# py-lidbox/lidbox

Measured on AMD Instinct MI355X. Metric: utterances/sec (16kHz x 2s) log-mel + x-vector train step, higher is better.
Workload: dtype f32; 1 GPU; log-mel + x-vector 4-lang train step, bs=256 per GPU, fp32 (BASELINE configs[1]); reference_model=lidbox.models.xvector, global_batch=256, per_gpu_batch=256, samples_per_utt=32000, frames=198, mel=40, languages=4, optimizer=Adam(1e-3, eps=1e-7), parallelism=dp1, grad_buckets=1, grad_sync=none, hip_graph=True, resident_batches=4, feature_prefetch=False

## Files before the change

### lidbox_amd/csrc/gemm.hip

```cpp
#include <stdlib.h>

#include <atomic>

#include "gemm_shared.h"
#include "gemm_sk.h"
#include <string.h>
#include "gemm_dma.h"
#include "gemm_dma8.h"
#include "gemm_tuned.h"

namespace {

constexpr int BK = 16;
#define LBX_ROWS_BOUNDS(BM, BN) __launch_bounds__(256, ((BM) * (BN) >= 16384 ? 3 : ((BM) * (BN) >= 8192 ? 6 : 8)))
#define LBX_TN_BOUNDS(BM, BN) __launch_bounds__(256, ((BM) * (BN) >= 16384 ? 3 : 1))

template <int ROWS, bool ALIGNED, int NT = 256>
struct KInnerLoader {
    static constexpr int F4R = BK / 4;
    static constexpr int RPP = NT / F4R;
    static constexpr int PASSES = ROWS >= RPP ? ROWS / RPP : 1;
    static constexpr bool PARTIAL = ROWS < RPP;
    static constexpr int LD = ROWS + 8 / F4R;
    float4 v[PASSES];
// ... 621 lines not shown

inline int dma_mode() {
    if (const char* e = getenv("LIDBOX_GEMM_DMA")) return atoi(e);
    return 1;
}

template <int BM, int BN, bool B_KINNER>
void launch_rows_dma_t(dim3 grid, hipStream_t st, RowsD Ad, const float* Bm, long ldb, RowsOutD Co, float* P, long m_beg, long m_end,
                       int K, int N, int epi, const float* aux, int tiles_n, unsigned ntiles, int kps, const DmaStream& sp, const ReduceJobs& rj) {
    hipLaunchKernelGGL((gemm_rows_dma_kernel<BM, BN, B_KINNER>), grid, dim3(256), 0, st, Ad, Bm, ldb, Co, P, m_beg, m_end, K, N, epi,
                       aux, tiles_n, ntiles, kps, sp, rj);
}

inline long carry_cap() {
    if (const char* e = getenv("LIDBOX_GEMM_CARRY_BLOCKS")) { const long v = atol(e); if (v >= 8) return v; }
    return 96;
}
struct Carry {
    const ReduceJob* jobs = nullptr;
    int njobs = 0;
    bool carried = false;
};

constexpr int DMA_STREAM_MIN_STEPS = 8;
constexpr int DMA_STREAM_MAX_G = 8;
struct DmaStreamPlan {
    int g = 0;
    long whole = 0, rem = 0;
    size_t ws_need = 0;
};
inline DmaStreamPlan dma_stream_plan(int bm, int bn, long M, int N, int K) {
    DmaStreamPlan pl;
    int force = -1;
    if (const char* e = getenv("LIDBOX_GEMM_STREAM_TAIL")) force = atoi(e);
    if (force == 0) return pl;
    const long tiles = lbx_cdiv(M, bm) * lbx_cdiv(N, bn);
    const long rem = tiles % NUM_CU;
    if (tiles < NUM_CU || rem == 0) return pl;
    const int nk = (int)lbx_cdiv(K, SK_BK);
    int best = 1;
    double best_cost = 1.0;
    for (int g = 2; g <= DMA_STREAM_MAX_G && nk / g >= DMA_STREAM_MIN_STEPS; ++g) {
        const double cost = (double)lbx_cdiv(rem * g, (long)NUM_CU) / g + 0.03 + 0.01 * g;
        if (cost < best_cost - 1e-9) { best_cost = cost; best = g; }
    }
    if (force > 1 && nk / force >= 2 && force <= 64) best = force;
    else if (best_cost > 0.9) return pl;
    if (best < 2) return pl;
    pl.g = best; pl.rem = rem; pl.whole = tiles - rem;
    pl.ws_need = SK_COUNTER_BYTES + (size_t)rem * best * bm * bn * sizeof(float);
    return pl;
}

template <bool B_KINNER>
int launch_rows_range(const RowsChoice& ch, bool al, RowsD Ad, const float* Bm, long ldb, RowsOutD Co, long m_beg,
                      long m_end, int K, int N, int epi, const float* aux, float* P, hipStream_t st, bool dma_ok = false,
                      const DmaStreamPlan* stream = nullptr, void* ws = nullptr, Carry* carry = nullptr) {
    const long Msub = m_end - m_beg;
    if (Msub <= 0) return LIDBOX_OK;
    const int tiles_n = (int)lbx_cdiv(N, ch.bn);
    const long ntiles = lbx_cdiv(Msub, ch.bm) * tiles_n;
    dim3 grid((unsigned)ntiles, (unsigned)ch.splits);
    if (g_last_launches[0] == 0) { g_first_tile[0] = ch.bm; g_first_tile[1] = ch.bn; }
    ++g_last_launches[(ch.bm == g_first_tile[0] && ch.bn == g_first_tile[1]) ? 0 : 1];
    if (ch.splits > 1) ++g_last_launches[2];
#define LBX_ROWS(BM_, BN_) launch_rows_t<BM_, BN_, B_KINNER>(al, grid, st, Ad, Bm, ldb, Co, P, m_beg, m_end, K, N, epi, aux, tiles_n, (unsigned)ntiles, ch.k_per_split)
#define LBX_ROWS8(BM_, BN_) launch_rows8_t<BM_, BN_, B_KINNER>(al, grid, st, Ad, Bm, ldb, Co, P, m_beg, m_end, K, N, epi, aux, tiles_n, (unsigned)ntiles, ch.k_per_split)
#define LBX_ROWS_DMA(BM_, BN_) launch_rows_dma_t<BM_, BN_, B_KINNER>(grid, st, Ad, Bm, ldb, Co, P, m_beg, m_end, K, N, epi, aux, tiles_n, ntiles_k, ch.k_per_split, sp, rj)
    if (dma_ok && al && dma_mode() != 0) {
        g_last_family = 1;
        DmaStream sp;
        const bool dma8 = ch.waves == 8 && ch.bm == 128;
        ReduceJobs rj;
        if (carry && !carry->carried && carry->njobs > 0) {
            rj = pack_carry(carry->jobs, carry->njobs, carry_cap());
            carry->carried = rj.total > 0;
        }
        unsigned ntiles_k = (unsigned)ntiles;
        if (stream && stream->g > 1 && ch.splits == 1) {
            sp.pieces = (unsigned)(stream->rem * stream->g);
            sp.npad = (sp.pieces + 7u) & ~7u;
            sp.g = stream->g;
            sp.first_tile = (unsigned)stream->whole;
            sp.epoch = sk_next_epoch();
            sp.counters = (unsigned*)ws;
            sp.slabs = (float*)((char*)ws + SK_COUNTER_BYTES);
            ntiles_k = (unsigned)stream->whole;
            grid.x = sp.npad + ntiles_k;
        }
        grid.x += rj.total;
        if (dma8) {
            g_last_family = 3;
            if (ch.bn == 128)
                hipLaunchKernelGGL((gemm_rows_dma8_kernel<128, B_KINNER>), grid, dim3(512), 0, st, Ad, Bm, ldb, Co, P, m_beg, m_end, K, N, epi, aux, tiles_n,
                                   ntiles_k, ch.k_per_split, sp, rj);
            else
                hipLaunchKernelGGL((gemm_rows_dma8_kernel<64, B_KINNER>), grid, dim3(512), 0, st, Ad, Bm, ldb, Co, P, m_beg, m_end, K, N, epi, aux, tiles_n,
                                   ntiles_k, ch.k_per_split, sp, rj);
        } else
        if (ch.bm == 128 && ch.bn == 128) LBX_ROWS_DMA(128, 128);
        else if (ch.bm == 128) LBX_ROWS_DMA(128, 64);
        else if (ch.bn == 128) LBX_ROWS_DMA(64, 128);
        else LBX_ROWS_DMA(64, 64);
    } else
    if (ch.waves == 8 && ch.bm == 128 && ch.bn == 128) LBX_ROWS8(128, 128);
    else if (ch.waves == 8 && ch.bm == 128 && ch.bn == 64) LBX_ROWS8(128, 64);
    else if (ch.bm == 128 && ch.bn == 128) LBX_ROWS(128, 128);
    else if (ch.bm == 128) LBX_ROWS(128, 64);
    else if (ch.bn == 128) LBX_ROWS(64, 128);
    else LBX_ROWS(64, 64);
#undef LBX_ROWS
#undef LBX_ROWS8
    LBX_LAUNCH_OK();
    if (ch.splits > 1) {
        long g = lbx_cdiv(Msub * N, 256);
        if (g > 2048) g = 2048;
        hipLaunchKernelGGL(rows_reduce_kernel, dim3((unsigned)g), dim3(256), 0, st, (const float*)P, ch.splits, m_beg,
                           Msub, N, Co, epi, aux);
        LBX_LAUNCH_OK();
    }
    return LIDBOX_OK;
}

inline int cand_index(int bm, int bn) { return bm == 128 ? (bn == 128 ? 0 : 1) : (bn == 128 ? 2 : 3); }

template <bool B_KINNER>
int launch_rows(lidbox_rows_t A, const float* Bm, long ldb, lidbox_rows_out_t Cd, int K, int N, int epi,
                const float* aux, void* ws, size_t ws_bytes, hipStream_t st, Carry* carry = nullptr) {
    const long M = (long)A.batch * A.rows_per_batch;
    g_last_launches[0] = g_last_launches[1] = g_last_launches[2] = 0;
    g_last_family = 0;
    if (M == 0 || N == 0) return LIDBOX_OK;
    const size_t wsb = ws ? ws_bytes : 0;
    const RowsChoice ch = choose_rows_env(B_KINNER ? 1 : 0, M, N, K, wsb);
    const bool al = rows_aligned(A) && K % 4 == 0 && aligned16(Bm) && ldb % 4 == 0 &&
                    (B_KINNER ? true : N % 4 == 0);
    RowsD Ad = to_dev(A);
    RowsOutD Co{Cd.base, Cd.batch_stride, Cd.row_stride, Cd.batch, Cd.rows_per_batch};
    float* P = (float*)ws;

    if (al && !getenv("LIDBOX_GEMM_PLAN") && aligned16(ws) && !sk_tuned_out(B_KINNER ? 1 : 0, M, N, K) &&
        sk_b_extent_ok(B_KINNER, K, N, ldb)) {
        const bool has_mask_ = epi == LIDBOX_EPI_RELU_MASK || epi == LIDBOX_EPI_ACCUM_RELU_MASK;
        const bool skp_ok = skp_mode() != 0 && (Cd.batch == 1 || Cd.rows_per_batch >= 32) && N % 4 == 0 && aligned16(Cd.base) &&
                            Cd.row_stride % 4 == 0 && (Cd.batch == 1 || Cd.batch_stride % 4 == 0) && (!has_mask_ || aligned16(aux)) &&
                            skp_policy(B_KINNER ? 1 : 0, M, N, K);
        if (skp_ok) {
            const SkRows sk = sk_rows_plan(B_KINNER ? 1 : 0, M, N, K, true);
            if (sk.ok && wsb >= sk.ws_need && sk_extent_ok(A, K)) {
                sk_set_lds_attr();
                g_last_launches[0] = 1;
                g_last_family = 2;
                g_first_tile[0] = SK_BM; g_first_tile[1] = SK_BN;
                unsigned* counters = (unsigned*)ws;
                float* slabs = (float*)((char*)ws + SK_COUNTER_BYTES);
                float* dummy = slabs + (size_t)sk.P * 2 * SK_SLAB;
                const bool has_mask = epi == LIDBOX_EPI_RELU_MASK || epi == LIDBOX_EPI_ACCUM_RELU_MASK;
                const bool accum = epi == LIDBOX_EPI_ACCUM || epi == LIDBOX_EPI_ACCUM_RELU_MASK || epi == LIDBOX_EPI_ACCUM_RELU;
                const unsigned ep = sk_next_epoch();
#define LBX_SKP(MASK_, ACC_)                                                                                                \
    hipLaunchKernelGGL((gemm_skp_rows_kernel<B_KINNER, MASK_, ACC_>), dim3(sk.P), dim3(256), (MASK_ || ACC_) ? SKP_LDS_BYTES : SK_LDS_BYTES, st, Ad, Bm, ldb, Co, M, K, \
                       N, epi, aux, sk.pl, ep, counters, slabs, dummy)
                if (has_mask && accum) LBX_SKP(true, true);
                else if (has_mask) LBX_SKP(true, false);
                else if (accum) LBX_SKP(false, true);
                else LBX_SKP(false, false);
#undef LBX_SKP
                LBX_LAUNCH_OK();
                return LIDBOX_OK;
            }
        }
        const SkRows sk = sk_rows_plan(B_KINNER ? 1 : 0, M, N, K);
        if (sk.ok && wsb >= sk.ws_need && sk_extent_ok(A, K)) {
            sk_set_lds_attr();
            g_last_launches[0] = 1;
            g_last_family = 2;
            g_first_tile[0] = SK_BM; g_first_tile[1] = SK_BN;
            unsigned* counters = (unsigned*)ws;
            float* slabs = (float*)((char*)ws + SK_COUNTER_BYTES);
            hipLaunchKernelGGL((gemm_sk_rows_kernel<B_KINNER>), dim3(sk.P), dim3(256), SK_LDS_BYTES, st, Ad, Bm, ldb, Co, M, K, N, epi,
                               aux, sk.pl, sk_next_epoch(), counters, slabs);
            LBX_LAUNCH_OK();
            return LIDBOX_OK;
        }
    }

    const bool dma_ok = al && sk_extent_ok(A, K) && sk_b_extent_ok(B_KINNER, K, N, ldb);
    if (dma_ok && dma_mode() != 0 && ch.splits == 1 && aligned16(ws)) {
        const DmaStreamPlan spl = dma_stream_plan(ch.bm, ch.bn, M, N, K);
        if (spl.g > 1 && wsb >= spl.ws_need)
            return launch_rows_range<B_KINNER>(ch, al, Ad, Bm, ldb, Co, 0, M, K, N, epi, aux, P, st, dma_ok, &spl, ws, carry);
    }
    const bool no_tail_split = ch.no_tail_split || getenv("LIDBOX_GEMM_NO_TAIL_SPLIT") != nullptr;
    if (!no_tail_split && ch.splits == 1) {
        const int tiles_n = (int)lbx_cdiv(N, ch.bn);
        const long tiles_m = lbx_cdiv(M, ch.bm);
        const long wgs = tiles_m * tiles_n;
        const long rounds = wgs / NUM_CU;
        if (rounds >= 1 && wgs % NUM_CU != 0) {
            const long main_tiles_m = rounds * NUM_CU / tiles_n;
            const long m_main = main_tiles_m * ch.bm;
            const long m_rem = M - m_main;
            if (main_tiles_m >= 1 && m_rem > 0) {
                const RowsChoice rem = choose_rows(B_KINNER ? 1 : 0, m_rem, N, K, wsb);
                const int c = cand_index(ch.bm, ch.bn), cr = cand_index(rem.bm, rem.bn);
                const double ksteps = (double)lbx_cdiv(K, BK);
                const double whole = launch_cost(c, wgs, ksteps);
                double split = launch_cost(c, main_tiles_m * tiles_n, ksteps) + 4.0 +
                               launch_cost(cr, lbx_cdiv(m_rem, rem.bm) * lbx_cdiv(N, rem.bn) * rem.splits,
                                           (double)rem.k_per_split / BK);
                if (rem.splits > 1) split += 5.0 + (double)m_rem * N * 4.0 * (rem.splits + 1) / 3.0e6;
                if (split < 0.97 * whole) {
                    int rc = launch_rows_range<B_KINNER>(ch, al, Ad, Bm, ldb, Co, 0, m_main, K, N, epi, aux, P, st, dma_ok, nullptr, nullptr, carry);
                    if (rc) return rc;
                    return launch_rows_range<B_KINNER>(rem, al, Ad, Bm, ldb, Co, m_main, M, K, N, epi, aux, P, st, dma_ok);
                }
            }
        }
    }
    return launch_rows_range<B_KINNER>(ch, al, Ad, Bm, ldb, Co, 0, M, K, N, epi, aux, P, st, dma_ok, nullptr, nullptr, carry);
}

struct TnPlan {
    int bm, bn, splits;
    long rows_per_split;
};

TnPlan tn_plan(long M, int K1, int N) {
    if (const char* f = getenv("LIDBOX_GEMM_TN_PLAN")) {
        int bm = 0, bn = 0;
        long sp = 0;
        if (sscanf(f, "%d,%d,%ld", &bm, &bn, &sp) == 3 && (bm == 64 || bm == 128) && (bn == 64 || bn == 128) && sp >= 1) {
            const long rps = lbx_cdiv(lbx_cdiv(M, sp), BK) * BK;
            return TnPlan{bm, bn, (int)lbx_cdiv(M, rps), rps};
        }
    }
    if (const TunedGemm* t = tuned_gemm(2, M, N, K1)) {
        const long rps = lbx_cdiv(lbx_cdiv(M, (long)t->splits), BK) * BK;
        return TnPlan{t->bm, t->bn, (int)lbx_cdiv(M, rps), rps};
    }
    TnPlan best{128, 128, 1, M};
    double best_cost = 1e30;
    for (int c = 0; c < 4; ++c) {
        const int bm = CAND[c][0], bn = CAND[c][1];
        const long tiles = lbx_cdiv(K1, bm) * lbx_cdiv(N, bn);
        for (long target = NUM_CU; target <= 8 * NUM_CU; target += NUM_CU / 2) {
            long s = target / tiles;
            if (s < 1) s = 1;
            const long max_s = lbx_cdiv(M, 4 * BK);
            if (s > max_s) s = max_s;
            if (s < 1) s = 1;
            long rps = lbx_cdiv(lbx_cdiv(M, s), BK) * BK;
            s = lbx_cdiv(M, rps);
            double cost = launch_cost(c, tiles * s, (double)rps / BK);
            cost += 5.0 + (double)K1 * N * 4.0 * (s + 1) / 3.0e6;
            if (cost < best_cost) { best_cost = cost; best = TnPlan{bm, bn, (int)s, rps}; }
        }
    }
    return best;
}

template <int BM, int BN>
void launch_tn_t(bool al, unsigned grid, hipStream_t st, RowsD A, RowsD Bd, float* P, float* Pc, long M, int K1, int N,
                 int tiles_n, int ntiles, long rps) {
    if (al)
        hipLaunchKernelGGL((gemm_tn_kernel<BM, BN, true>), dim3(grid), dim3(256), 0, st, A, Bd, P, Pc, M, K1, N, tiles_n,
                           ntiles, rps);
    else
        hipLaunchKernelGGL((gemm_tn_kernel<BM, BN, false>), dim3(grid), dim3(256), 0, st, A, Bd, P, Pc, M, K1, N, tiles_n,
                           ntiles, rps);
}

}
// ... 1 lines not shown
extern "C" int lidbox_gemm_plan_query(int kind, long M, int N, int K, size_t workspace_bytes, int* out4) {
    LBX_ARG(out4 && M > 0 && N > 0 && K > 0 && kind >= 0 && kind <= 2, "kind in {0 nn, 1 nt, 2 tn}, positive sizes");
    if (kind == 2) {
        const TnPlan pl = tn_plan(M, K, N);
        out4[0] = pl.bm; out4[1] = pl.bn; out4[2] = pl.splits; out4[3] = (int)pl.rows_per_split;
    } else {
        const RowsChoice ch = choose_rows_env(kind, M, N, K, workspace_bytes);
        out4[0] = ch.bm; out4[1] = ch.bn; out4[2] = ch.splits; out4[3] = ch.k_per_split;
    }
    return LIDBOX_OK;
}

extern "C" int lidbox_gemm_plan_is_stream_k(int kind, long M, int N, int K, size_t workspace_bytes) {
    if (M <= 0 || N <= 0 || K <= 0 || kind < 0 || kind > 2) return 0;
    if (kind == 2) {
        const SkTn t = sk_tn_plan(M, K, N);
        return t.ok && workspace_bytes >= t.ws_need && !sk_tuned_out(2, M, N, K);
    }
    {
        const SkRows r = sk_rows_plan(kind, M, N, K);
        return r.ok && workspace_bytes >= r.ws_need && (kind == 1 || N % 4 == 0) && !sk_tuned_out(kind, M, N, K);
    }
    return LIDBOX_OK;
}

extern "C" int lidbox_gemm_plan_waves(int kind, long M, int N, int K, size_t workspace_bytes) {
    if (M <= 0 || N <= 0 || K <= 0 || kind < 0 || kind > 1) return 4;
    return choose_rows_env(kind, M, N, K, workspace_bytes).waves;
}

extern "C" int lidbox_gemm_last_family(void) { return g_last_family; }

extern "C" int lidbox_gemm_plan_stream_tail(int kind, long M, int N, int K, size_t workspace_bytes) {
    if (M <= 0 || N <= 0 || K <= 0 || kind < 0 || kind > 1 || dma_mode() == 0) return 0;
    if (!getenv("LIDBOX_GEMM_PLAN") && lidbox_gemm_plan_is_stream_k(kind, M, N, K, workspace_bytes)) return 0;
    const RowsChoice ch = choose_rows_env(kind, M, N, K, workspace_bytes);
    if (ch.splits != 1) return 0;
    const DmaStreamPlan spl = dma_stream_plan(ch.bm, ch.bn, M, N, K);
    return (spl.g > 1 && workspace_bytes >= spl.ws_need) ? spl.g : 0;
}

extern "C" int lidbox_gemm_last_launches(int* out3) {
    LBX_ARG(out3, "out3 != NULL");
    out3[0] = g_last_launches[0]; out3[1] = g_last_launches[1]; out3[2] = g_last_launches[2];
    return LIDBOX_OK;
}

extern "C" size_t lidbox_gemm_rows_workspace(long M, int N, int K) {
    if (M <= 0 || N <= 0 || K <= 0) return 0;
    size_t need = 0;
    for (int kind = 0; kind < 2; ++kind) {
        const RowsChoice ch = choose_rows(kind, M, N, K, (size_t)64 << 20);
        if (ch.splits > 1 && (size_t)ch.splits * M * N * sizeof(float) > need) need = (size_t)ch.splits * M * N * sizeof(float);
    }
    for (int bm = 64; bm <= 128; bm += 64)
        for (int bn = 64; bn <= 128; bn += 64) {
            const DmaStreamPlan spl = dma_stream_plan(bm, bn, M, N, K);
            if (spl.g > 1 && spl.ws_need > need) need = spl.ws_need;
        }
    for (int kind = 0; kind < 2; ++kind) {
        const SkRows sk = sk_rows_plan(kind, M, N, K);
        if (sk.ok && sk.ws_need > need) need = sk.ws_need;
        if (skp_mode() != 0 && skp_policy(kind, M, N, K)) {
            const SkRows skp = sk_rows_plan(kind, M, N, K, true);
            if (skp.ok && skp.ws_need > need) need = skp.ws_need;
        }
    }
    return need;
}

extern "C" int lidbox_gemm_nn(lidbox_rows_t A, const float* Bm, long ldb, lidbox_rows_out_t C, int K, int N,
                              int epilogue, const float* aux, void* workspace, size_t workspace_bytes,
                              lidbox_stream_t stream) {
    if (validate_rows_call(__func__, A, Bm, ldb, C, K, N, epilogue, aux, N)) return LIDBOX_E_INVALID;
    return launch_rows<false>(A, Bm, ldb, C, K, N, epilogue, aux, workspace, workspace_bytes, (hipStream_t)stream);
}


extern "C" int lidbox_gemm_nt(lidbox_rows_t A, const float* Bm, long ldb, lidbox_rows_out_t C, int K, int N,
                              int epilogue, const float* aux, void* workspace, size_t workspace_bytes,
                              lidbox_stream_t stream) {
    if (validate_rows_call(__func__, A, Bm, ldb, C, K, N, epilogue, aux, K)) return LIDBOX_E_INVALID;
    return launch_rows<true>(A, Bm, ldb, C, K, N, epilogue, aux, workspace, workspace_bytes, (hipStream_t)stream);
}

extern "C" size_t lidbox_gemm_tn_workspace(int M, int K1, int N) {
    if (M <= 0 || K1 <= 0 || N <= 0) return 0;
    const TnPlan pl = tn_plan(M, K1, N);
    size_t need = ((size_t)pl.splits * K1 * N + (size_t)pl.splits * N) * sizeof(float);
    const SkTn sk = sk_tn_plan(M, K1, N);
    if (sk.ok && sk.ws_need > need) need = sk.ws_need;
    return need;
}

namespace {

int tn_partial_launch(const char* fn, lidbox_rows_t A, lidbox_rows_t Bd, float* Cm, long ldc, int K1, int N, int accumulate,
                      float* bias_grad, void* workspace, size_t workspace_bytes, hipStream_t st, ReduceJob* job) {
    *job = ReduceJob{};
    if (check_rows(fn, A.base, A.batch_stride, A.row_stride, A.batch, A.rows_per_batch)) return LIDBOX_E_INVALID;
    if (check_rows(fn, Bd.base, Bd.batch_stride, Bd.row_stride, Bd.batch, Bd.rows_per_batch)) return LIDBOX_E_INVALID;
    LBX_ARG(Cm && K1 >= 1 && N >= 1 && ldc >= N, "C != NULL, K1, N >= 1, ldc >= N");
    const long M = (long)A.batch * A.rows_per_batch;
    LBX_ARG(M == (long)Bd.batch * Bd.rows_per_batch, "A and B row counts differ");
    LBX_ARG(M >= 1, "M >= 1");
    auto finish = [&](const float* P, const float* Pc, int splits) {
// ... 168 lines not shown
    if (ch_out) *ch_out = ch;
    if (pl_out) *pl_out = pl;
    return true;
}

extern "C" int lidbox_gemm_nt_tn_carry(lidbox_rows_t dY, const float* W, long ldb, lidbox_rows_out_t dX, int Co, int N, int epilogue,
                                       const float* aux, void* ws_nt, size_t ws_nt_bytes, lidbox_rows_t X, float* dW, long ldc, int K1,
                                       int accumulate, float* bias_grad, void* ws_tn, size_t ws_tn_bytes,
                                       const lidbox_reduce_job_t* jobs, int njobs, lidbox_reduce_job_t* job_out, lidbox_stream_t stream) {
    hipStream_t st = (hipStream_t)stream;
    if (job_out) memset(job_out, 0, sizeof *job_out);
    ReduceJob pend[MAX_CARRY];
    const int npend = jobs_in(jobs, njobs, pend);
    LBX_ARG(npend >= 0 && npend < MAX_CARRY, "at most 1 non-empty pending job per call");
    for (int i = 0; i < npend; ++i)
        LBX_ARG((const void*)pend[i].P != ws_nt && (const void*)pend[i].P != ws_tn, "a pending job's slices live in this call's workspaces");
    for (int i = 0; i < npend; ++i) LBX_ARG(pend[i].splits >= 0, "an optimizer-prepare job runs through lidbox_reduce_jobs_run only");
    const long M = (long)dY.batch * dY.rows_per_batch;
    bool pair = dma_mode() != 0 && getenv("LIDBOX_GEMM_NO_PAIR") == nullptr && M >= 1 && N >= 1 && K1 >= 1 && Co >= 1 && W && dW && ws_tn &&
                ws_nt != ws_tn;
    if (pair) {
        if (validate_rows_call(__func__, dY, W, ldb, dX, Co, N, epilogue, aux, Co)) return LIDBOX_E_INVALID;
        if (check_rows(__func__, X.base, X.batch_stride, X.row_stride, X.batch, X.rows_per_batch)) return LIDBOX_E_INVALID;
        LBX_ARG((long)X.batch * X.rows_per_batch == M && ldc >= Co, "X and dY row counts differ, or ldc < Co");
    }
    RowsChoice ch{};
    TnPlan pl{};
    if (pair) {
        const size_t wsb = ws_nt ? ws_nt_bytes : 0;
        const bool al_rows = rows_aligned(dY) && aligned16(W) && ldb % 4 == 0 && sk_extent_ok(dY, Co) && sk_b_extent_ok(true, Co, N, ldb) &&
                             aligned16(ws_nt);
        const bool al_tn = rows_aligned(X) && sk_extent_ok(X, K1) && aligned16(ws_tn);
        pair = al_rows && al_tn && pair_plan(M, Co, N, K1, wsb, ws_tn_bytes, &ch, &pl);
    }
    if (!pair) {
        lidbox_reduce_job_t all[MAX_CARRY];
        for (int i = 0; i < npend; ++i) memcpy(&all[i], &pend[i], sizeof(ReduceJob));
        int rc = lidbox_gemm_tn_partial(X, dY, dW, ldc, K1, Co, accumulate, bias_grad, ws_tn, ws_tn_bytes, &all[npend], stream);
        if (rc) return rc;
        if (ws_nt == ws_tn) {
            rc = lidbox_reduce_jobs_run(all, npend + 1, stream);
            if (rc) return rc;
            return lidbox_gemm_nt(dY, W, ldb, dX, Co, N, epilogue, aux, ws_nt, ws_nt_bytes, stream);
        }
        return lidbox_gemm_nt_carry(dY, W, ldb, dX, Co, N, epilogue, aux, ws_nt, ws_nt_bytes, all, npend + 1, stream);
    }
    PairRows r;
    r.A = to_dev(dY); r.Bm = W; r.ldb = ldb;
    r.Cd = RowsOutD{dX.base, dX.batch_stride, dX.row_stride, dX.batch, dX.rows_per_batch};
    r.P = (float*)ws_nt; r.M = M; r.K = Co; r.N = N; r.epi = epilogue; r.aux = aux;
    r.tiles_n = (int)lbx_cdiv((long)N, 64L);
    r.ntiles = (unsigned)(lbx_cdiv(M, 64L) * r.tiles_n);
    r.k_per_split = ch.k_per_split; r.nx = r.ntiles; r.partial = ch.splits > 1 ? 1 : 0;
    if (ch.splits == 1 && ws_nt) {
        const DmaStreamPlan spl = dma_stream_plan(64, 64, M, N, Co);
        if (spl.g > 1 && ws_nt_bytes >= spl.ws_need) {
            r.sp.pieces = (unsigned)(spl.rem * spl.g);
            r.sp.npad = (r.sp.pieces + 7u) & ~7u;
            r.sp.g = spl.g;
            r.sp.first_tile = (unsigned)spl.whole;
            r.sp.epoch = sk_next_epoch();
            r.sp.counters = (unsigned*)ws_nt;
            r.sp.slabs = (float*)((char*)ws_nt + SK_COUNTER_BYTES);
            r.ntiles = (unsigned)spl.whole;
            r.nx = r.sp.npad + r.ntiles;
        }
    }
    PairTn t;
    t.A = to_dev(X); t.Bd = to_dev(dY);
    t.P = (float*)ws_tn; t.Pc = bias_grad ? t.P + (size_t)pl.splits * K1 * Co : nullptr;
    t.M = M; t.K1 = K1; t.N = Co; t.tiles_n = (int)lbx_cdiv((long)Co, 64L);
    t.ntiles = (int)(lbx_cdiv((long)K1, 64L) * t.tiles_n);
    t.rows_per_split = pl.rows_per_split;
    const unsigned rows_blocks = r.nx * (unsigned)ch.splits;
    ReduceJobs rj;
    if (npend > 0 && getenv("LIDBOX_GEMM_NO_CARRY") == nullptr) rj = pack_carry(pend, npend, carry_cap());
    const unsigned grid = rj.total + rows_blocks + (unsigned)(t.ntiles * pl.splits);
    g_last_launches[0] = 1; g_last_launches[1] = 0; g_last_launches[2] = (job_out ? 0 : 1) + (ch.splits > 1 ? 1 : 0);
    g_last_family = 1;
    g_last_carried = rj.total > 0 ? npend : 0;
    hipLaunchKernelGGL(gemm_nt_tn_pair_kernel, dim3(grid), dim3(256), 0, st, r, t, rows_blocks, rj);
    LBX_LAUNCH_OK();
    if (npend > 0 && rj.total == 0) {
        int rc = run_reduce_jobs(pend, npend, st);
        if (rc) return rc;
    }
    if (ch.splits > 1) {
        long g = lbx_cdiv(M * N, 256);
        if (g > 2048) g = 2048;
        hipLaunchKernelGGL(rows_reduce_kernel, dim3((unsigned)g), dim3(256), 0, st, (const float*)r.P, ch.splits, 0L, M, N, r.Cd, epilogue,
                           aux);
        LBX_LAUNCH_OK();
    }
    if (job_out && reduce_job_vec_ok(t.P, t.Pc, pl.splits, (long)K1 * Co, Co, dW, ldc, bias_grad)) {
        const ReduceJob j = make_reduce_job(t.P, t.Pc, pl.splits, (long)K1 * Co, Co, dW, ldc, accumulate, bias_grad);
        memcpy(job_out, &j, sizeof j);
        return LIDBOX_OK;
    }
    launch_splitk_reduce((const float*)t.P, (const float*)t.Pc, pl.splits, (long)K1 * Co, Co, dW, ldc, accumulate, bias_grad, st);
    LBX_LAUNCH_OK();
    return LIDBOX_OK;
}

extern "C" int lidbox_gemm_nt_tn(lidbox_rows_t dY, const float* W, long ldb, lidbox_rows_out_t dX, int Co, int N, int epilogue,
                                 const float* aux, void* ws_nt, size_t ws_nt_bytes, lidbox_rows_t X, float* dW, long ldc, int K1,
                                 int accumulate, float* bias_grad, void* ws_tn, size_t ws_tn_bytes, lidbox_stream_t stream) {
    return lidbox_gemm_nt_tn_carry(dY, W, ldb, dX, Co, N, epilogue, aux, ws_nt, ws_nt_bytes, X, dW, ldc, K1, accumulate, bias_grad, ws_tn,
                                   ws_tn_bytes, nullptr, 0, nullptr, stream);
}

extern "C" int lidbox_gemm_plan_is_pair(long M, int Co, int N, int K1, size_t ws_nt_bytes, size_t ws_tn_bytes) {
    return pair_plan(M, Co, N, K1, ws_nt_bytes, ws_tn_bytes, nullptr, nullptr) ? 1 : 0;
}

extern "C" size_t lidbox_colsum_workspace(long M, int N) {
    long slices = lbx_cdiv(M, 256);
    if (slices > 128) slices = 128;
    if (slices < 1) slices = 1;
    return (size_t)slices * N * sizeof(float);
}

extern "C" int lidbox_colsum(lidbox_rows_t A, int N, float* out, int accumulate, void* workspace,
                             size_t workspace_bytes, lidbox_stream_t stream) {
    if (check_rows(__func__, A.base, A.batch_stride, A.row_stride, A.batch, A.rows_per_batch)) return LIDBOX_E_INVALID;
    LBX_ARG(out && N >= 1, "out != NULL, N >= 1");
    const long M = (long)A.batch * A.rows_per_batch;
    long slices = lbx_cdiv(M, 256);
    if (slices > 128) slices = 128;
    if (slices < 1) slices = 1;
    LBX_ARG(workspace && workspace_bytes >= (size_t)slices * N * sizeof(float), "workspace too small (lidbox_colsum_workspace)");
    const long rps = lbx_cdiv(M, slices);
    hipStream_t st = (hipStream_t)stream;
    hipLaunchKernelGGL(colsum_stage1, dim3((unsigned)lbx_cdiv(N, 64), (unsigned)slices), dim3(256), 0, st,
                       to_dev(A), M, N, rps, (float*)workspace);
    LBX_LAUNCH_OK();
    hipLaunchKernelGGL(colsum_stage2, dim3((unsigned)lbx_cdiv(N, 256)), dim3(256), 0, st, (const float*)workspace,
                       (int)slices, N, out, accumulate);
    LBX_LAUNCH_OK();
    return LIDBOX_OK;
}
// ... 1 lines not shown
```

### lidbox_amd/csrc/gemm_dma.h

```cpp
#pragma once

#include "gemm_sk.h"

namespace {

constexpr int DMA_STAGES = 3;

template <int ROWS>
struct DmaInner {
    static constexpr int PW = ROWS / 64;
    const float* sb;
    unsigned vo[PW];
    int rd;
    __device__ __forceinline__ void init(const float* base, const long (&roff)[PW], int k0, int lane, int wsub) {
        sb = sk_uniform(base + k0);
        const int chunk = (lane & 3) ^ ((lane >> 4) & 3);
#pragma unroll
        for (int i = 0; i < PW; ++i) vo[i] = (unsigned)((roff[i] + chunk * 4) * 4);
        rd = (wsub * (ROWS / 2) + (lane & 31)) * 16;
    }
    __device__ __forceinline__ void issue(int i, unsigned dst) const { sk_dma_s(sb, vo[i], dst); }
    __device__ __forceinline__ void issue_tail(int i, unsigned dst, int kvalid, int lane) const {
        const int chunk = (lane & 3) ^ ((lane >> 4) & 3);
        const float* p = reinterpret_cast<const float*>(reinterpret_cast<const char*>(sb) + vo[i]);
// ... 13 lines not shown

template <int COLS>
struct DmaOuter {
    static constexpr int PW = COLS / 64;
    static constexpr int LPR = COLS / 4;
    static constexpr int RPP = 64 / LPR;
    const float* sb;
    unsigned vo[PW];
    long step;
    int rd;
    __device__ __forceinline__ void init(const float* base, long ld, int col0, int ncols, int k0, int lane, int wv, int wsub) {
        sb = sk_uniform(base + (long)k0 * ld + col0);
        int c = (lane % LPR) * 4;
        if (col0 + c >= ncols) c = 0;
#pragma unroll
        for (int i = 0; i < PW; ++i) vo[i] = (unsigned)(((long)(RPP * (wv * PW + i) + lane / LPR) * ld + c) * 4);
        step = (long)SK_BK * ld;
        rd = (4 * (lane >> 5)) * COLS + wsub * (COLS / 2) + (lane & 31);
    }
    __device__ __forceinline__ void issue(int i, unsigned dst) const { sk_dma_s(sb, vo[i], dst); }
    __device__ __forceinline__ void issue_tail(int i, unsigned dst, int kvalid, int lane, int wv) const {
        const float* p = reinterpret_cast<const float*>(reinterpret_cast<const char*>(sb) + vo[i]);
        sk_dma_f(RPP * (wv * PW + i) + lane / LPR < kvalid ? p : g_sk_zero, dst);
    }
    __device__ __forceinline__ void advance() { sb += step; }
    template <int NB>
    __device__ __forceinline__ void read(const float* st, int lane, int s2, float (&v)[NB][4]) const {
#pragma unroll
        for (int b = 0; b < NB; ++b)
#pragma unroll
            for (int j = 0; j < 4; ++j) v[b][j] = st[rd + (8 * s2 + j) * COLS + b * 32];
    }
};

template <int MI, int NJ, int J0, int J1>
__device__ __forceinline__ void dma_mma(const float (&a)[MI][4], const float (&b)[NJ][4], f32x16 (&acc)[MI][NJ]) {
#pragma unroll
    for (int j = J0; j < J1; ++j)
#pragma unroll
        for (int bi = 0; bi < MI; ++bi)
#pragma unroll
            for (int bj = 0; bj < NJ; ++bj)
                acc[bi][bj] = __builtin_amdgcn_mfma_f32_32x32x2f32(a[bi][j], b[bj][j], acc[bi][bj], 0, 0, 0);
}

struct DmaStream {
    unsigned npad = 0;
    unsigned pieces = 0;
    int g = 1;
    unsigned first_tile = 0;
    unsigned epoch = 0;
    unsigned* counters = nullptr;
    float* slabs = nullptr;
};

template <int MI, int NJ>
__device__ __forceinline__ void dma_slab_store(float* slab, const f32x16 (&acc)[MI][NJ], int wv, int lane) {
    const __amdgpu_buffer_rsrc_t r = __builtin_amdgcn_make_buffer_rsrc(const_cast<float*>(sk_uniform(slab)), 0, MI * NJ * 4096 * 4, 0x00020000);
#pragma unroll
    for (int bi = 0; bi < MI; ++bi)
#pragma unroll
        for (int bj = 0; bj < NJ; ++bj)
#pragma unroll
            for (int r4 = 0; r4 < 4; ++r4) {
                const f32x4_t x = {acc[bi][bj][4 * r4], acc[bi][bj][4 * r4 + 1], acc[bi][bj][4 * r4 + 2], acc[bi][bj][4 * r4 + 3]};
                __builtin_amdgcn_raw_buffer_store_b128(__builtin_bit_cast(u32x4_t, x), r,
                                                       ((((wv * (MI * NJ) + bi * NJ + bj) * 4 + r4) * 64 + lane) * 4) * 4, 0,  16);
            }
}
template <int MI, int NJ>
__device__ __forceinline__ void dma_slab_add(const float* slab, f32x16 (&acc)[MI][NJ], int wv, int lane) {
    const __amdgpu_buffer_rsrc_t r = __builtin_amdgcn_make_buffer_rsrc(const_cast<float*>(sk_uniform(slab)), 0, MI * NJ * 4096 * 4, 0x00020000);
#pragma unroll
    for (int bi = 0; bi < MI; ++bi)
#pragma unroll
        for (int bj = 0; bj < NJ; ++bj) {
#pragma unroll
            for (int r4 = 0; r4 < 4; ++r4) {
                const f32x4_t x = __builtin_bit_cast(
                    f32x4_t, __builtin_amdgcn_raw_buffer_load_b128(r, ((((wv * (MI * NJ) + bi * NJ + bj) * 4 + r4) * 64 + lane) * 4) * 4, 0,  16));
#pragma unroll
                for (int j = 0; j < 4; ++j) acc[bi][bj][4 * r4 + j] += x[j];
            }
            __builtin_amdgcn_sched_barrier(0);
        }
}

template <int BM, int BN, bool B_KINNER>
__device__ __forceinline__ void rows_dma_body(const RowsD& A, const float* __restrict__ Bm, long ldb, const RowsOutD& Cd, float* __restrict__ P,
                                              long m_beg, long M, int K, int N, int epi, const float* __restrict__ aux, int tiles_n,
                                              unsigned ntiles, int k_per_split, const DmaStream& sp, unsigned bx, unsigned by, int partial,
                                              float* smem) {
    constexpr int MI = BM / 64, NJ = BN / 64;
    constexpr int A_ST = BM * SK_BK, B_ST = SK_BK * BN, ST = A_ST + B_ST;
    constexpr int PA = BM / 64, PB = BN / 64;

    const int tid = threadIdx.x, lane = tid & 63;
    const int wv = __builtin_amdgcn_readfirstlane(tid >> 6);
    const int wm = wv >> 1, wn = wv & 1;
    const unsigned lds0 = __builtin_amdgcn_readfirstlane((unsigned)(size_t)(__attribute__((address_space(3))) void*)smem);
    const int split = (int)by;
    unsigned chunk;
    int kbeg, kend, part = -1;
    unsigned rem_t = 0;
    if (bx < sp.npad) {
        if (bx >= sp.pieces) return;
        rem_t = bx / (unsigned)sp.g;
        part = (int)(bx - rem_t * (unsigned)sp.g);
        chunk = sp.first_tile + rem_t;
        const int nk = (K + SK_BK - 1) / SK_BK;
        kbeg = (part * nk / sp.g) * SK_BK;
        kend = min(K, ((part + 1) * nk / sp.g) * SK_BK);
    } else {
        chunk = xcd_chunk_id(bx - sp.npad, ntiles);
        kbeg = split * k_per_split;
        kend = min(K, kbeg + k_per_split);
    }
    const int tn = chunk % tiles_n;
    const long m0 = m_beg + (long)(chunk / tiles_n) * BM;
    const int n0 = tn * BN;
    const int n = (kend - kbeg + SK_BK - 1) / SK_BK;
    const int ktail = kend - kbeg - (n - 1) * SK_BK;

    DmaInner<BM> oa;
    {
        long roff[PA];
#pragma unroll
        for (int i = 0; i < PA; ++i) {
            long r = m0 + 16 * (wv * PA + i) + (lane >> 2);
            if (r >= M) r = m0;
            roff[i] = row_offset(A, (unsigned)r);
        }
        oa.init(A.base, roff, kbeg, lane, wm);
    }
    DmaInner<BN> obi;
    DmaOuter<BN> obo;
    if (B_KINNER) {
        long roff[PB];
#pragma unroll
        for (int i = 0; i < PB; ++i) {
            long r = n0 + 16 * (wv * PB + i) + (lane >> 2);
            if (r >= N) r = n0;
            roff[i] = r * ldb;
        }
        obi.init(Bm, roff, kbeg, lane, wn);
    } else {
        obo.init(Bm, ldb, n0, N, kbeg, lane, wv, wn);
    }
    f32x16 acc[MI][NJ];
#pragma unroll
    for (int i = 0; i < MI; ++i)
#pragma unroll
        for (int j = 0; j < NJ; ++j)
#pragma unroll
            for (int r = 0; r < 16; ++r) acc[i][j][r] = 0.f;

    auto issue = [&](int pc, int step, int stage) {
        const bool tail = step == n - 1 && ktail < SK_BK;
        if (pc < PA) {
            const unsigned d = lds0 + (unsigned)((stage * ST + (wv * PA + pc) * 256) * 4);
            if (tail) oa.issue_tail(pc, d, ktail, lane);
            else oa.issue(pc, d);
        } else {
            const int q = pc - PA;
            const unsigned d = lds0 + (unsigned)((stage * ST + A_ST + (wv * PB + q) * 256) * 4);
            if (B_KINNER) { if (tail) obi.issue_tail(q, d, ktail, lane); else obi.issue(q, d); }
            else { if (tail) obo.issue_tail(q, d, ktail, lane, wv); else obo.issue(q, d); }
        }
    };
// ... 17 lines not shown
        }
    if (n >= DMA_STAGES - 1) sk_wait_vm<(DMA_STAGES - 2) * NP>();
    else sk_wait_vm<0>();
    __builtin_amdgcn_s_barrier();
    float a0[MI][4], b0[NJ][4], a1[MI][4], b1[NJ][4];
    if (n > 0) {
        ra(smem, 0, a0);
        rb(smem + A_ST, 0, b0);
    }
    int cur = 0;
    for (int t = 0; t < n; ++t) {
        if (t + 1 < n) {
            if (DMA_STAGES >= 4 && t + DMA_STAGES - 2 < n) sk_wait_vm<(DMA_STAGES >= 4 ? (DMA_STAGES - 3) * NP : 0)>();
            else sk_wait_vm<0>();
        }
        __builtin_amdgcn_s_barrier();
        int nxt = cur + 1;
        if (nxt == DMA_STAGES) nxt = 0;
        const bool more = t + DMA_STAGES - 1 < n;
        int tgt = cur + DMA_STAGES - 1;
        if (tgt >= DMA_STAGES) tgt -= DMA_STAGES;
        const float* st = smem + cur * ST;
        dma_mma<MI, NJ, 0, 1>(a0, b0, acc);
        __builtin_amdgcn_sched_barrier(0);
        ra(st, 1, a1);
        rb(st + A_ST, 1, b1);
        __builtin_amdgcn_sched_barrier(0);
        dma_mma<MI, NJ, 1, 2>(a0, b0, acc);
        if (more) issue(0, t + DMA_STAGES - 1, tgt);
        __builtin_amdgcn_sched_barrier(0);
        dma_mma<MI, NJ, 2, 3>(a0, b0, acc);
        if (more) issue(1, t + DMA_STAGES - 1, tgt);
        __builtin_amdgcn_sched_barrier(0);
        dma_mma<MI, NJ, 3, 4>(a0, b0, acc);
        if (more && NP > 2) issue(2, t + DMA_STAGES - 1, tgt);
        __builtin_amdgcn_sched_barrier(0);
        dma_mma<MI, NJ, 0, 1>(a1, b1, acc);
        if (more) {
            if (NP > 3) issue(3, t + DMA_STAGES - 1, tgt);
            next();
        }
        __builtin_amdgcn_sched_barrier(0);
        if (t + 1 < n) {
            const float* sn = smem + nxt * ST;
            ra(sn, 0, a0);
            rb(sn + A_ST, 0, b0);
        }
        __builtin_amdgcn_sched_barrier(0);
        dma_mma<MI, NJ, 1, 4>(a1, b1, acc);
        cur = nxt;
    }
    if (part >= 0) {
        constexpr int SLAB = BM * BN;
        dma_slab_store<MI, NJ>(sp.slabs + (size_t)bx * SLAB, acc, wv, lane);
        asm volatile("s_waitcnt vmcnt(0)" ::: "memory");
        __syncthreads();
        unsigned* flag = reinterpret_cast<unsigned*>(smem);
        if (tid == 0) {
            unsigned old = __hip_atomic_load(sp.counters + rem_t, __ATOMIC_RELAXED, __HIP_MEMORY_SCOPE_AGENT);
            unsigned cnt;
            for (;;) {
                cnt = (old >> 8) == sp.epoch ? (old & 255u) : 0u;
                if (__hip_atomic_compare_exchange_strong(sp.counters + rem_t, &old, (sp.epoch << 8) | (cnt + 1u), __ATOMIC_RELAXED,
                                                         __ATOMIC_RELAXED, __HIP_MEMORY_SCOPE_AGENT))
                    break;
            }
            *flag = cnt;
        }
        __syncthreads();
        if (*flag != (unsigned)(sp.g - 1)) return;
#pragma unroll
        for (int i = 0; i < MI; ++i)
#pragma unroll
            for (int j = 0; j < NJ; ++j)
#pragma unroll
                for (int r = 0; r < 16; ++r) acc[i][j][r] = 0.f;
        for (int q = 0; q < sp.g; ++q)
            dma_slab_add<MI, NJ>(sp.slabs + ((size_t)rem_t * sp.g + q) * SLAB, acc, wv, lane);
        if (tid == 0) __hip_atomic_store(sp.counters + rem_t, 0u, __ATOMIC_RELAXED, __HIP_MEMORY_SCOPE_AGENT);
    }
    store_rows_tile<MI, NJ>(acc, m0, n0, wm, wn, lane, m_beg, M, N, epi, aux, Cd, P, split, 0ull, false, nullptr, nullptr, partial);
}

template <int BM, int BN>
constexpr int dma_stage_floats() { return (BM + BN) * SK_BK; }

template <int BM, int BN, bool B_KINNER>
__global__ __launch_bounds__(256, (BM * BN >= 16384 ? 3 : (BM * BN >= 8192 ? 4 : 6))) void gemm_rows_dma_kernel(
    RowsD A, const float* __restrict__ Bm, long ldb, RowsOutD Cd, float* __restrict__ P, long m_beg, long M, int K, int N, int epi,
    const float* __restrict__ aux, int tiles_n, unsigned ntiles, int k_per_split, DmaStream sp, ReduceJobs rj) {
    __shared__ __attribute__((aligned(16))) float smem[DMA_STAGES * dma_stage_floats<BM, BN>()];
    if (blockIdx.x < rj.total) {
        if (blockIdx.y == 0) reduce_jobs_run(rj, blockIdx.x);
        return;
    }
    rows_dma_body<BM, BN, B_KINNER>(A, Bm, ldb, Cd, P, m_beg, M, K, N, epi, aux, tiles_n, ntiles, k_per_split, sp, blockIdx.x - rj.total,
                                    blockIdx.y, gridDim.y > 1 ? 1 : 0, smem);
}

template <int COLS>
struct DmaOuterRows {
    static constexpr int PW = COLS / 64;
    static constexpr int LPR = COLS / 4;
    static constexpr int RPP = 64 / LPR;
    const float* sb;
    int off[PW];
    unsigned tt[PW];
    int a_step, a_wrap;
    unsigned rpb;
    int mleft[PW];
    int rd;

    __device__ __forceinline__ void init(const RowsD& X, int col0, int ncols, long mbeg, long mend, int lane, int wv, int wsub) {
        sb = sk_uniform(X.base + col0);
        int c = (lane % LPR) * 4;
        if (col0 + c >= ncols) c = 0;
        a_step = (int)(SK_BK * X.rs);
        a_wrap = X.batch == 1 ? 0 : (int)(X.bs - (long)X.rpb * X.rs);
        rpb = X.batch == 1 ? 0xffffffffu : (unsigned)X.rpb;
#pragma unroll
        for (int i = 0; i < PW; ++i) {
            const long m = mbeg + RPP * (wv * PW + i) + lane / LPR;
            const unsigned bq = X.batch == 1 ? 0u : (unsigned)m / rpb;
            tt[i] = (unsigned)m - (X.batch == 1 ? 0u : bq * rpb);
            off[i] = (int)((long)bq * X.bs + (long)tt[i] * X.rs) + c;
            mleft[i] = (int)(mend - m);
        }
        rd = (4 * (lane >> 5)) * COLS + wsub * (COLS / 2) + (lane & 31);
    }
    __device__ __forceinline__ void issue(int i, unsigned dst, bool tail) {
        if (!tail) {
            sk_dma_s(sb, (unsigned)off[i] * 4u, dst);
        } else {
            const float* p = reinterpret_cast<const float*>(reinterpret_cast<const char*>(sb) + (size_t)((unsigned)off[i] * 4u));
            sk_dma_f(mleft[i] > 0 ? p : g_sk_zero, dst);
        }
        mleft[i] -= SK_BK;
        tt[i] += SK_BK;
        off[i] += a_step;
        while (tt[i] >= rpb) { tt[i] -= rpb; off[i] += a_wrap; }
    }
    template <int NB>
    __device__ __forceinline__ void read(const float* st, int lane, int s2, float (&v)[NB][4]) const {
#pragma unroll
        for (int b = 0; b < NB; ++b)
#pragma unroll
            for (int j = 0; j < 4; ++j) v[b][j] = st[rd + (8 * s2 + j) * COLS + b * 32];
    }
};

// ... 151 lines not shown
```

Baseline: 120,200 utterances/s.

## Finish split-K reduction in-kernel via atomic counters instead of separate reduce launch

For 64x64 split-K DMA GEMM launches, each split writes its partial tile into a per-tile slab, and the last split to arrive (found through an epoch-tagged atomic counter) sums all slabs and runs the epilogue. This removes the separate rows_reduce_kernel launch and its full partial-buffer pass. It adds a batched slab-sum helper and requires a larger workspace sizing path. The cost is atomics, serialized summation in the last-arriving block, and extra slab traffic.

Result: slower. 117,400 utterances/s (-2.4%).

```diff
diff --git a/lidbox_amd/csrc/gemm.hip b/lidbox_amd/csrc/gemm.hip
--- a/lidbox_amd/csrc/gemm.hip
+++ b/lidbox_amd/csrc/gemm.hip
@@ -697,10 +697,22 @@
     return pl;
 }
 
+inline size_t split_finish_ws(long tiles, int splits) { return SK_COUNTER_BYTES + (size_t)tiles * splits * 64 * 64 * sizeof(float); }
+inline bool split_finish_ok(const RowsChoice& ch, long tiles, const void* ws, size_t ws_bytes) {
+    return ch.splits > 1 && ch.splits <= 250 && ch.bm == 64 && ch.bn == 64 && ch.waves != 8 && ws && aligned16(ws) &&
+           (size_t)tiles * sizeof(unsigned) <= SK_COUNTER_BYTES && ws_bytes >= split_finish_ws(tiles, ch.splits);
+}
+inline void split_finish_arm(DmaStream& sp, int splits, void* ws) {
+    sp.g = splits;
+    sp.epoch = sk_next_epoch();
+    sp.counters = (unsigned*)ws;
+    sp.slabs = (float*)((char*)ws + SK_COUNTER_BYTES);
+}
+
 template <bool B_KINNER>
 int launch_rows_range(const RowsChoice& ch, bool al, RowsD Ad, const float* Bm, long ldb, RowsOutD Co, long m_beg,
                       long m_end, int K, int N, int epi, const float* aux, float* P, hipStream_t st, bool dma_ok = false,
-                      const DmaStreamPlan* stream = nullptr, void* ws = nullptr, Carry* carry = nullptr) {
+                      const DmaStreamPlan* stream = nullptr, void* ws = nullptr, Carry* carry = nullptr, size_t ws_bytes = 0) {
     const long Msub = m_end - m_beg;
     if (Msub <= 0) return LIDBOX_OK;
     const int tiles_n = (int)lbx_cdiv(N, ch.bn);
@@ -708,7 +720,7 @@
     dim3 grid((unsigned)ntiles, (unsigned)ch.splits);
     if (g_last_launches[0] == 0) { g_first_tile[0] = ch.bm; g_first_tile[1] = ch.bn; }
     ++g_last_launches[(ch.bm == g_first_tile[0] && ch.bn == g_first_tile[1]) ? 0 : 1];
-    if (ch.splits > 1) ++g_last_launches[2];
+    bool reduce = ch.splits > 1;
 #define LBX_ROWS(BM_, BN_) launch_rows_t<BM_, BN_, B_KINNER>(al, grid, st, Ad, Bm, ldb, Co, P, m_beg, m_end, K, N, epi, aux, tiles_n, (unsigned)ntiles, ch.k_per_split)
 #define LBX_ROWS8(BM_, BN_) launch_rows8_t<BM_, BN_, B_KINNER>(al, grid, st, Ad, Bm, ldb, Co, P, m_beg, m_end, K, N, epi, aux, tiles_n, (unsigned)ntiles, ch.k_per_split)
 #define LBX_ROWS_DMA(BM_, BN_) launch_rows_dma_t<BM_, BN_, B_KINNER>(grid, st, Ad, Bm, ldb, Co, P, m_beg, m_end, K, N, epi, aux, tiles_n, ntiles_k, ch.k_per_split, sp, rj)
@@ -732,6 +744,9 @@
             sp.slabs = (float*)((char*)ws + SK_COUNTER_BYTES);
             ntiles_k = (unsigned)stream->whole;
             grid.x = sp.npad + ntiles_k;
+        } else if (split_finish_ok(ch, ntiles, P, ws_bytes)) {
+            split_finish_arm(sp, ch.splits, P);
+            reduce = false;
         }
         grid.x += rj.total;
         if (dma8) {
@@ -757,7 +772,8 @@
 #undef LBX_ROWS
 #undef LBX_ROWS8
     LBX_LAUNCH_OK();
-    if (ch.splits > 1) {
+    if (reduce) {
+        ++g_last_launches[2];
         long g = lbx_cdiv(Msub * N, 256);
         if (g > 2048) g = 2048;
         hipLaunchKernelGGL(rows_reduce_kernel, dim3((unsigned)g), dim3(256), 0, st, (const float*)P, ch.splits, m_beg,
@@ -858,12 +874,12 @@
                 if (split < 0.97 * whole) {
                     int rc = launch_rows_range<B_KINNER>(ch, al, Ad, Bm, ldb, Co, 0, m_main, K, N, epi, aux, P, st, dma_ok, nullptr, nullptr, carry);
                     if (rc) return rc;
-                    return launch_rows_range<B_KINNER>(rem, al, Ad, Bm, ldb, Co, m_main, M, K, N, epi, aux, P, st, dma_ok);
+                    return launch_rows_range<B_KINNER>(rem, al, Ad, Bm, ldb, Co, m_main, M, K, N, epi, aux, P, st, dma_ok, nullptr, nullptr, nullptr, wsb);
                 }
             }
         }
     }
-    return launch_rows_range<B_KINNER>(ch, al, Ad, Bm, ldb, Co, 0, M, K, N, epi, aux, P, st, dma_ok, nullptr, nullptr, carry);
+    return launch_rows_range<B_KINNER>(ch, al, Ad, Bm, ldb, Co, 0, M, K, N, epi, aux, P, st, dma_ok, nullptr, nullptr, carry, wsb);
 }
 
 struct TnPlan {
@@ -971,6 +987,10 @@
     for (int kind = 0; kind < 2; ++kind) {
         const RowsChoice ch = choose_rows(kind, M, N, K, (size_t)64 << 20);
         if (ch.splits > 1 && (size_t)ch.splits * M * N * sizeof(float) > need) need = (size_t)ch.splits * M * N * sizeof(float);
+        if (ch.splits > 1 && ch.bm == 64 && ch.bn == 64) {
+            const size_t fin = split_finish_ws(lbx_cdiv(M, 64L) * lbx_cdiv((long)N, 64L), ch.splits);
+            if (fin > need) need = fin;
+        }
     }
     for (int bm = 64; bm <= 128; bm += 64)
         for (int bn = 64; bn <= 128; bn += 64) {
@@ -1245,6 +1265,11 @@
     r.tiles_n = (int)lbx_cdiv((long)N, 64L);
     r.ntiles = (unsigned)(lbx_cdiv(M, 64L) * r.tiles_n);
     r.k_per_split = ch.k_per_split; r.nx = r.ntiles; r.partial = ch.splits > 1 ? 1 : 0;
+    const bool finish = split_finish_ok(ch, (long)r.ntiles, ws_nt, ws_nt ? ws_nt_bytes : 0);
+    if (finish) {
+        split_finish_arm(r.sp, ch.splits, ws_nt);
+        r.partial = 0;
+    }
     if (ch.splits == 1 && ws_nt) {
         const DmaStreamPlan spl = dma_stream_plan(64, 64, M, N, Co);
         if (spl.g > 1 && ws_nt_bytes >= spl.ws_need) {
@@ -1269,7 +1294,7 @@
     ReduceJobs rj;
     if (npend > 0 && getenv("LIDBOX_GEMM_NO_CARRY") == nullptr) rj = pack_carry(pend, npend, carry_cap());
     const unsigned grid = rj.total + rows_blocks + (unsigned)(t.ntiles * pl.splits);
-    g_last_launches[0] = 1; g_last_launches[1] = 0; g_last_launches[2] = (job_out ? 0 : 1) + (ch.splits > 1 ? 1 : 0);
+    g_last_launches[0] = 1; g_last_launches[1] = 0; g_last_launches[2] = (job_out ? 0 : 1) + (ch.splits > 1 && !finish ? 1 : 0);
     g_last_family = 1;
     g_last_carried = rj.total > 0 ? npend : 0;
     hipLaunchKernelGGL(gemm_nt_tn_pair_kernel, dim3(grid), dim3(256), 0, st, r, t, rows_blocks, rj);
@@ -1278,7 +1303,7 @@
         int rc = run_reduce_jobs(pend, npend, st);
         if (rc) return rc;
     }
-    if (ch.splits > 1) {
+    if (ch.splits > 1 && !finish) {
         long g = lbx_cdiv(M * N, 256);
         if (g > 2048) g = 2048;
         hipLaunchKernelGGL(rows_reduce_kernel, dim3((unsigned)g), dim3(256), 0, st, (const float*)r.P, ch.splits, 0L, M, N, r.Cd, epilogue,
diff --git a/lidbox_amd/csrc/gemm_dma.h b/lidbox_amd/csrc/gemm_dma.h
--- a/lidbox_amd/csrc/gemm_dma.h
+++ b/lidbox_amd/csrc/gemm_dma.h
@@ -89,6 +89,7 @@
     unsigned epoch = 0;
     unsigned* counters = nullptr;
     float* slabs = nullptr;
+    __host__ __device__ bool finishes_splits() const { return npad == 0 && g > 1; }
 };
 
 template <int MI, int NJ>
@@ -104,6 +105,42 @@
                 __builtin_amdgcn_raw_buffer_store_b128(__builtin_bit_cast(u32x4_t, x), r,
                                                        ((((wv * (MI * NJ) + bi * NJ + bj) * 4 + r4) * 64 + lane) * 4) * 4, 0,  16);
             }
+}
+constexpr int DMA_SUM_BATCH = 3;
+__device__ __forceinline__ void dma_slab_sum(const float* slab0, size_t stride, int g, f32x16 (&acc)[1][1], int wv, int lane) {
+    const unsigned lo = (unsigned)(((wv * 4) * 64 + lane) * 16);
+#pragma unroll
+    for (int r = 0; r < 16; ++r) acc[0][0][r] = 0.f;
+    auto rsrc = [&](int q) {
+        return __builtin_amdgcn_make_buffer_rsrc(const_cast<float*>(sk_uniform(slab0 + (size_t)q * stride)), 0, 4096 * 4, 0x00020000);
+    };
+    auto load = [&](int q, f32x4_t (&x)[4]) {
+        const __amdgpu_buffer_rsrc_t r = rsrc(q);
+#pragma unroll
+        for (int r4 = 0; r4 < 4; ++r4)
+            x[r4] = __builtin_bit_cast(f32x4_t, __builtin_amdgcn_raw_buffer_load_b128(r, lo + (unsigned)(r4 * 64 * 16), 0,  16));
+    };
+    auto add = [&](const f32x4_t (&x)[4]) {
+#pragma unroll
+        for (int r4 = 0; r4 < 4; ++r4)
+#pragma unroll
+            for (int j = 0; j < 4; ++j) acc[0][0][4 * r4 + j] += x[r4][j];
+    };
+    int q = 0;
+    for (; q + DMA_SUM_BATCH <= g; q += DMA_SUM_BATCH) {
+        f32x4_t x[DMA_SUM_BATCH][4];
+#pragma unroll
+        for (int i = 0; i < DMA_SUM_BATCH; ++i) load(q + i, x[i]);
+        __builtin_amdgcn_sched_barrier(0);
+#pragma unroll
+        for (int i = 0; i < DMA_SUM_BATCH; ++i) add(x[i]);
+        __builtin_amdgcn_sched_barrier(0);
+    }
+    for (; q < g; ++q) {
+        f32x4_t x0[4];
+        load(q, x0);
+        add(x0);
+    }
 }
 template <int MI, int NJ>
 __device__ __forceinline__ void dma_slab_add(const float* slab, f32x16 (&acc)[MI][NJ], int wv, int lane) {
@@ -152,6 +189,10 @@
         chunk = xcd_chunk_id(bx - sp.npad, ntiles);
         kbeg = split * k_per_split;
         kend = min(K, kbeg + k_per_split);
+        if (sp.finishes_splits()) {
+            rem_t = chunk;
+            part = split;
+        }
     }
     const int tn = chunk % tiles_n;
     const long m0 = m_beg + (long)(chunk / tiles_n) * BM;
@@ -275,7 +316,7 @@
     }
     if (part >= 0) {
         constexpr int SLAB = BM * BN;
-        dma_slab_store<MI, NJ>(sp.slabs + (size_t)bx * SLAB, acc, wv, lane);
+        dma_slab_store<MI, NJ>(sp.slabs + ((size_t)rem_t * sp.g + part) * SLAB, acc, wv, lane);
         asm volatile("s_waitcnt vmcnt(0)" ::: "memory");
         __syncthreads();
         unsigned* flag = reinterpret_cast<unsigned*>(smem);
@@ -292,14 +333,23 @@
         }
         __syncthreads();
         if (*flag != (unsigned)(sp.g - 1)) return;
-#pragma unroll
-        for (int i = 0; i < MI; ++i)
-#pragma unroll
-            for (int j = 0; j < NJ; ++j)
-#pragma unroll
-                for (int r = 0; r < 16; ++r) acc[i][j][r] = 0.f;
-        for (int q = 0; q < sp.g; ++q)
-            dma_slab_add<MI, NJ>(sp.slabs + ((size_t)rem_t * sp.g + q) * SLAB, acc, wv, lane);
+        bool summed = false;
+        if constexpr (MI * NJ == 1) {
+            if (sp.finishes_splits()) {
+                dma_slab_sum(sp.slabs + (size_t)rem_t * sp.g * SLAB, SLAB, sp.g, acc, wv, lane);
+                summed = true;
+            }
+        }
+        if (!summed) {
+#pragma unroll
+            for (int i = 0; i < MI; ++i)
+#pragma unroll
+                for (int j = 0; j < NJ; ++j)
+#pragma unroll
+                    for (int r = 0; r < 16; ++r) acc[i][j][r] = 0.f;
+            for (int q = 0; q < sp.g; ++q)
+                dma_slab_add<MI, NJ>(sp.slabs + ((size_t)rem_t * sp.g + q) * SLAB, acc, wv, lane);
+        }
         if (tid == 0) __hip_atomic_store(sp.counters + rem_t, 0u, __ATOMIC_RELAXED, __HIP_MEMORY_SCOPE_AGENT);
     }
     store_rows_tile<MI, NJ>(acc, m0, n0, wm, wn, lane, m_beg, M, N, epi, aux, Cd, P, split, 0ull, false, nullptr, nullptr, partial);
@@ -318,7 +368,7 @@
         return;
     }
     rows_dma_body<BM, BN, B_KINNER>(A, Bm, ldb, Cd, P, m_beg, M, K, N, epi, aux, tiles_n, ntiles, k_per_split, sp, blockIdx.x - rj.total,
-                                    blockIdx.y, gridDim.y > 1 ? 1 : 0, smem);
+                                    blockIdx.y, (gridDim.y > 1 && !sp.finishes_splits()) ? 1 : 0, smem);
 }
 
 template <int COLS>
```
